# UZ-SLAMLab/DefSLAM

Measured on AMD Instinct MI355X. Metric: SfT GN iters/sec (500-node mesh, 1k matches), higher is better.
Workload: dtype f64

## Files before the change

### defslam_amd/csrc/sft_batch.h

```cpp
#pragma once

#define SFTB_NW 8
#ifndef SFTB_LIN_NW
#define SFTB_LIN_NW 8
#endif
#ifndef SFTB_LIN_WAVES
#define SFTB_LIN_WAVES 2
#endif
#ifndef SFTB_TRIAL_WAVES
#define SFTB_TRIAL_WAVES 2
#endif

__device__ __forceinline__ void sftb_ctl_lds(char* smem, Ctl*& ctl, double*& red, double*& out, double*& panel) {
  ctl = reinterpret_cast<Ctl*>(smem);
  red = reinterpret_cast<double*>(smem + 512);
  out = red + 16 * 27 + 5;
  panel = out + 32;
}

__global__ __launch_bounds__(64 * SFTB_NW, 2) void sftb_init_kernel(const SftDev* __restrict__ probs, SftRun* __restrict__ runs, int* __restrict__ counters, int* __restrict__ lin_list, int tail_below) {
  const SftDev& P = probs[blockIdx.x];
  if (blockIdx.x == 0 && threadIdx.x == 0 && (int)gridDim.x <= tail_below) counters[6] = 1;
  init_state<64 * SFTB_NW>(P);
  if (threadIdx.x == 0) {
    SftRun& R = runs[blockIdx.x];
    R.lambda = -1.0; R.ni = 2.0; R.chi_cur = 0.0; R.chi_ini = 0.0; R.rho = 0.0; R.lambda_start = 0.0;
    R.it = 0; R.qmax = 0; R.nbad = 0; R.accepted = 0; R.all_ok = 1; R.iters = 0; R.trials = 0; R.fact_ok = 1;
    R.state = P.max_iters > 0 ? SFTB_LIN : SFTB_FINISH;
    if (P.max_iters > 0) lin_list[atomicAdd(&counters[2], 1)] = blockIdx.x;
  }
}

template <int NW>
__device__ __forceinline__ void sftb_lin_problem(const SftDev& P, SftRun& R, Ctl* ctl, double* red, double* out, double* panel) {
  constexpr int NT = 64 * NW;
  const int tid = threadIdx.x;
  auto nothing = [] {};
  const double chi0 = linearise<NW, decltype(nothing), true>(P, ctl, red, out, panel, nothing);
  double lambda = R.lambda;
  if (R.it == 0) {
    double mx = 0.0;
    for (int r = tid; r < P.Dn; r += NT) mx = fmax(mx, fabs(h_diag(P, r)));
    if (tid < 6) mx = fmax(mx, fabs(P.Hcorner[tid * 8]));
    mx = block_max(mx, red);
    lambda = 1e-5 * mx;
  }
  if (tid == 0) {
    if (R.it == 0) { R.lambda = lambda; R.ni = 2.0; R.nbad = 0; }
    R.chi_cur = chi0; R.chi_ini = chi0; R.qmax = 0; R.rho = 0.0; R.accepted = 0; R.all_ok = 1; R.lambda_start = lambda;
    R.state = SFTB_TRIAL;
  }
}

__global__ __launch_bounds__(64 * SFTB_LIN_NW, SFTB_LIN_WAVES) void sftb_lin_kernel(const SftDev* __restrict__ probs, SftRun* __restrict__ runs, int* __restrict__ counters,
                                                                                  const int* __restrict__ lin_list, int B, int tail_below) {
  constexpr int NW = SFTB_LIN_NW, NT = 64 * NW;
  extern __shared__ __attribute__((aligned(16))) char smem[];
  __shared__ int next_b;
  Ctl* ctl; double *red, *out, *panel;
  sftb_ctl_lds(smem, ctl, red, out, panel);
  const int tid = threadIdx.x;
  if (counters[6] || B - counters[0] <= tail_below) {
    if (blockIdx.x == 0 && tid == 0) counters[6] = 1;
    return;
  }
  if (blockIdx.x == 0 && tid == 0) counters[7]++;
  auto fetch = [&]() { const int i = atomicAdd(&counters[3], 1); return i < counters[2] ? lin_list[i] : -1; };
  int nxt = -1;
  if (tid == 0) nxt = fetch();
  while (true) {
    if (tid == 0) next_b = nxt;
    __syncthreads();
    const int b = __builtin_amdgcn_readfirstlane(next_b);
    if (b < 0) break;
    if (tid == 0) { nxt = fetch(); atomicAdd(&counters[9], 1); }
    sftb_lin_problem<NW>(probs[b], runs[b], ctl, red, out, panel);
  }
}

__global__ __launch_bounds__(64, 1) void sftb_factor_kernel(const SftDev* __restrict__ probs, SftRun* __restrict__ runs, int* __restrict__ counters, int B) {
  extern __shared__ __attribute__((aligned(16))) char smem[];
  lds_double* lds = to_lds(reinterpret_cast<double*>(smem));
  const int lane = threadIdx.x;
  if (counters[6]) return;
  for (int i = lane; i < WV_LDS_DOUBLES; i += 64) lds[i] = 0.0;
  if (blockIdx.x == 0 && lane == 0) { counters[2] = 0; counters[3] = 0; }
  WvPrev Q;
  Q.Lg = nullptr; Q.Linv = nullptr; Q.x = nullptr; Q.nT = 0; Q.active = 0; Q.xb = 0.0;
  int n_done = 0;
  while (true) {
    int b = 0;
    if (lane == 0) b = atomicAdd(&counters[1], 1);
    b = __builtin_amdgcn_readfirstlane(b);
    if (b >= B) break;
    if (runs[b].state != SFTB_TRIAL) continue;
    const SftDev& P = probs[b];
    const double lambda = runs[b].lambda;
    double xcam;
    const int ok = wv_factor(P, lambda, lambda, lds, Q, xcam);
    if (lane == 0) runs[b].fact_ok = ok;
    Q = wv_prev_of(P, ok, xcam, lane);
    n_done++;
  }
  int lane_now;
  asm volatile("v_mbcnt_lo_u32_b32 %0, -1, 0\n\tv_mbcnt_hi_u32_b32 %0, -1, %0" : "=v"(lane_now));
  if (Q.active) wv_backsub_now(Q, lane_now);
  if (lane_now == 0 && n_done) atomicAdd(&counters[8], n_done);
}

template <int NW>
__device__ __forceinline__ int sftb_trial_problem(const SftDev& P, SftRun& R, Ctl* ctl, double* red, double* out, double* panel, int* counters, int* lin_list, int b) {
  constexpr int NT = 64 * NW;
  const int tid = threadIdx.x;
  const int Dn = P.Dn;
  const int Dnp = ((Dn + NB - 1) / NB) * NB;
  const int ok = R.fact_ok;
  const double lam = R.lambda;
  const bool in_lds = P.lds_class >= 1;
  if (!in_lds)
    for (int i = tid; i < 3 * P.n; i += NT) {
      const double v = P.xyz[i];
      P.xyz_bak[i] = v;
      const int a = P.act[i / 3];
      if (a >= 0) P.xyz[i] = v + P.x[3 * a + (i % 3)];
    }
  if (tid < 7) R.pose_bak[tid] = P.pose[tid];
  __syncthreads();
  if (tid == 0) pose_oplus(P.pose, P.x + Dnp);
  double sc = 0.0;
  for (int r = tid; r < Dn; r += NT) { const double xv = P.x[r]; sc += xv * (lam * xv + P.Hbord[(size_t)6 * Dnp + r]); }
  if (tid < 6) { const double xv = P.x[Dnp + tid]; sc += xv * (lam * xv + P.Hcorner[42 + tid]); }
  __syncthreads();
  block_sum<1>(&sc, red, out);
  const double scale = out[0];
  __syncthreads();
  const auto staged = asm_records<NW, 1>(P, panel);
  const double chi_new = in_lds ? eval_edges<false, 1>(P, ctl, red, out, staged, P.x)
                                : eval_edges<false, 0>(P, ctl, red, out, asm_records<NW, 0>(P, panel));
  if (tid == 0) {
    const double tempChi = ok ? chi_new : DBL_MAX;
    double rho = (R.chi_cur - tempChi);
    rho /= (scale + 1e-3);
    R.rho = rho;
    if (rho > 0 && isfinite(tempChi)) {
      double alpha = 1. - pow((2 * rho - 1), 3);
      alpha = fmin(alpha, 2. / 3.);
      const double sf = fmax(1. / 3., alpha);
      R.lambda = lam * sf; R.ni = 2.0; R.chi_cur = tempChi; R.accepted = 1;
      ctl->stop = 0;
    } else {
      R.lambda = lam * R.ni; R.ni *= 2.0;
      ctl->stop = 1;
    }
    R.qmax++;
    R.all_ok &= ok;
    ctl->qmax = R.qmax;
    ctl->rho = rho;
  }
  __syncthreads();
  if (ctl->stop) {
    if (!in_lds)
      for (int i = tid; i < 3 * P.n; i += NT) P.xyz[i] = P.xyz_bak[i];
    if (tid < 7) P.pose[tid] = R.pose_bak[tid];
  } else if (in_lds) {
    for (int i = tid; i < 3 * P.n; i += NT) P.xyz[i] = staged.xyz_l[i];
  }
  const bool again = (ctl->rho < 0) && (ctl->qmax < 10);
  if (again) return 0;
  __syncthreads();
  if (tid == 0) {
    const int qmax = R.qmax;
    R.trials += qmax;
    R.iters++;
    if (P.trace) {
      double* t = P.trace + R.it * 8;
      t[0] = R.chi_ini; t[1] = R.lambda_start; t[2] = qmax; t[3] = R.chi_cur; t[4] = R.lambda; t[5] = R.rho; t[6] = R.accepted; t[7] = R.all_ok;
    }
    if (!R.all_ok) P.res->status |= 1;
    bool term = (qmax == 10) || (R.rho == 0);
    if (!term) {
      if ((R.chi_ini - R.chi_cur) * 1e3 < R.chi_ini) R.nbad++; else R.nbad = 0;
      term = R.nbad >= 3;
    }
    R.it++;
    if (R.it >= P.max_iters) term = true;
    ctl->nbad = term ? 1 : 0;
    ctl->it = R.iters;
    ctl->accepted = R.trials;
    R.state = term ? SFTB_DONE : SFTB_LIN;
    if (!term && lin_list) lin_list[atomicAdd(&counters[2], 1)] = b;
  }
  __syncthreads();
  if (ctl->nbad) {
    const int iters = ctl->it, trials = ctl->accepted;
    __syncthreads();
    classify<NT>(P, ctl, panel, iters, trials);
    if (tid == 0) atomicAdd(&counters[0], 1);
    return 2;
  }
  return 1;
}

__global__ __launch_bounds__(64 * SFTB_NW, SFTB_TRIAL_WAVES) void sftb_trial_kernel(const SftDev* __restrict__ probs, SftRun* __restrict__ runs, int* __restrict__ counters, int* __restrict__ lin_list) {
  constexpr int NW = SFTB_NW, NT = 64 * NW;
  SftRun& R = runs[blockIdx.x];
  const int st = R.state;
  if (counters[6]) return;
  if (blockIdx.x == 0 && threadIdx.x == 0) counters[1] = 0;
  if (st != SFTB_TRIAL && st != SFTB_FINISH) return;
  extern __shared__ __attribute__((aligned(16))) char smem[];
  const SftDev& P = probs[blockIdx.x];
  Ctl* ctl; double *red, *out, *panel;
  sftb_ctl_lds(smem, ctl, red, out, panel);
  const int tid = threadIdx.x;
  if (st == SFTB_FINISH) {
    classify<NT>(P, ctl, panel, 0, 0);
    if (tid == 0) { R.state = SFTB_DONE; atomicAdd(&counters[0], 1); }
    return;
  }
  (void)sftb_trial_problem<NW>(P, R, ctl, red, out, panel, counters, lin_list, blockIdx.x);
}

__device__ __noinline__ void sftb_solve8(const SftDev& P, unsigned ctl_off, unsigned ws_off, double lambda) {
  typedef __attribute__((address_space(3))) char lds_char;
  Ctl* ctl = reinterpret_cast<Ctl*>((char*)(lds_char*)(size_t)__builtin_amdgcn_readfirstlane(ctl_off));
  double* ws = reinterpret_cast<double*>((char*)(lds_char*)(size_t)__builtin_amdgcn_readfirstlane(ws_off));
  factor_tiles_df8<1>(P, ctl, ws, lambda, true);
  backsub_tiles<8>(P, ctl, ws);
}

__global__ __launch_bounds__(64 * SFTB_NW, SFT_WAVES_PER_EU) void sftb_tail_kernel(const SftDev* __restrict__ probs, SftRun* __restrict__ runs, int* __restrict__ counters, int B, int tail_below) {
  constexpr int NW = SFTB_NW, NT = 64 * NW;
  extern __shared__ __attribute__((aligned(16))) char smem[];
  Ctl* ctl; double *red, *out, *panel;
  sftb_ctl_lds(smem, ctl, red, out, panel);
  const int tid = threadIdx.x;
  if (!counters[6]) {
    if (B - counters[0] > tail_below) return;
    if (blockIdx.x == 0 && tid == 0) counters[6] = 1;
  }
  while (true) {
    __syncthreads();
    if (tid == 0) ctl->it = atomicAdd(&counters[5], 1);
    __syncthreads();
    const int b = __builtin_amdgcn_readfirstlane(ctl->it);
    __syncthreads();
    if (b >= B) break;
    SftRun& R = runs[b];
    const SftDev& P = probs[b];
    int st = R.state;
    if (st == SFTB_FINISH) {
      classify<NT>(P, ctl, panel, 0, 0);
      if (tid == 0) { R.state = SFTB_DONE; atomicAdd(&counters[0], 1); }
      continue;
    }
    while (st == SFTB_LIN || st == SFTB_TRIAL) {
      if (st == SFTB_LIN) {
        sftb_lin_problem<NW>(P, R, ctl, red, out, panel);
        __syncthreads();
// ... 13 lines not shown
```

### defslam_amd/csrc/sft_wave.h

```cpp
#pragma once

#if defined(WV_STEP_TRACE) && defined(DSH_LAB)
#define WV_T_DECL long long wv_tr[9] = {0, 0, 0, 0, 0, 0, 0, 0, 0}, wv_tl = clock64()
#define WV_T(e) do { const long long t__ = clock64(); wv_tr[e] += t__ - wv_tl; wv_tl = t__; } while (0)
#define WV_T_ARG , long long (&wv_tr)[9], long long& wv_tl
#define WV_T_PASS , wv_tr, wv_tl
#define WV_T_DUMP(P) do { if ((threadIdx.x & 63) == 0) for (int e__ = 0; e__ < 9; e__++) (P).dbg[40 + e__] = (double)wv_tr[e__]; } while (0)
#else
#define WV_T_DECL do {} while (0)
#define WV_T(e) do {} while (0)
#define WV_T_ARG
#define WV_T_PASS
#define WV_T_DUMP(P) do {} while (0)
#endif

__host__ __device__ constexpr int wv_phys(int r, int d) {
  return d == 0 ? r : (d <= 3 ? 8 * d + r : (d == 4 ? 32 + (r & 3) : 8 * (8 - d) + ((r + 8 - d) & 7)));
}
constexpr int WV_AGPR_TILES = 32;
constexpr int WV_L_WIN = 0;
constexpr int WV_L_BORD = 1024;
constexpr int WV_L_WSCR = 2048;
constexpr int WV_L_CN = 2336;
constexpr int WV_L_XRING = 2400;
// ... 32 lines not shown
               "v_mfma_f64_16x16x4_f64 %0, %2, a[%c7:%c8], %0\n\t"
               "v_mfma_f64_16x16x4_f64 %0, %3, a[%c9:%c10], %0\n\t"
               "v_mfma_f64_16x16x4_f64 %0, %4, a[%c11:%c12], %0"
               : "=&v"(Y)
               : "v"(Wt[0]), "v"(Wt[1]), "v"(Wt[2]), "v"(Wt[3]), "i"(8 * T), "i"(8 * T + 1), "i"(8 * T + 2), "i"(8 * T + 3), "i"(8 * T + 4), "i"(8 * T + 5),
                 "i"(8 * T + 6), "i"(8 * T + 7)
               : "memory");
}
__device__ __forceinline__ void wv_trsm_vgpr(v4d& Y, const v4d& Wt, const v4d& D, int q0 = 0) {
  if (q0 <= 0) {
    asm volatile("s_nop 1\n\t"
                 "v_mfma_f64_16x16x4_f64 %0, %1, %5, 0\n\t"
                 "v_mfma_f64_16x16x4_f64 %0, %2, %6, %0\n\t"
                 "v_mfma_f64_16x16x4_f64 %0, %3, %7, %0\n\t"
                 "v_mfma_f64_16x16x4_f64 %0, %4, %8, %0"
                 : "=&v"(Y)
                 : "v"(Wt[0]), "v"(Wt[1]), "v"(Wt[2]), "v"(Wt[3]), "v"(D[0]), "v"(D[1]), "v"(D[2]), "v"(D[3])
                 : "memory");
  } else {
    asm volatile("s_nop 1\n\tv_mfma_f64_16x16x4_f64 %0, %1, %2, 0" : "=&v"(Y) : "v"(Wt[3]), "v"(D[3]) : "memory");
    if (q0 <= 2) asm volatile("v_mfma_f64_16x16x4_f64 %0, %1, %2, %0" : "+v"(Y) : "v"(Wt[2]), "v"(D[2]) : "memory");
    if (q0 <= 1) asm volatile("v_mfma_f64_16x16x4_f64 %0, %1, %2, %0" : "+v"(Y) : "v"(Wt[1]), "v"(D[1]) : "memory");
  }
}
struct WvTri { double a[10]; };
__device__ __forceinline__ void wv_tri_load(const lds_double* wscr, int lane, WvTri& A) {
  const lds_double* p = wscr + (lane & 3) * 17 + (lane >> 4);
#pragma unroll
  for (int q = 0; q < 4; q++)
#pragma unroll
    for (int k = 0; k <= q; k++) A.a[q * (q + 1) / 2 + k] = p[68 * q + 4 * k];
}
#define WV_TRI_BODY(D0, D1, D2, D3)                          \
  "v_mfma_f64_4x4x4_4b_f64 %3, %10, " D0 ", 0\n\t"   \
  "v_mfma_f64_4x4x4_4b_f64 %2, %7, " D0 ", 0\n\t"    \
  "v_mfma_f64_4x4x4_4b_f64 %3, %11, " D1 ", %3\n\t"  \
  "v_mfma_f64_4x4x4_4b_f64 %2, %8, " D1 ", %2\n\t"   \
  "v_mfma_f64_4x4x4_4b_f64 %3, %12, " D2 ", %3\n\t"  \
  "v_mfma_f64_4x4x4_4b_f64 %2, %9, " D2 ", %2\n\t"   \
  "v_mfma_f64_4x4x4_4b_f64 %3, %13, " D3 ", %3\n\t"  \
  "v_mfma_f64_4x4x4_4b_f64 %1, %5, " D0 ", 0\n\t"    \
  "v_mfma_f64_4x4x4_4b_f64 %0, %4, " D0 ", 0\n\t"    \
  "v_mfma_f64_4x4x4_4b_f64 %1, %6, " D1 ", %1"
template <int T>
__device__ __forceinline__ void wv_trsm4_agpr(v4d& Y, const WvTri& A) {
  asm volatile(WV_TRI_BODY("a[%c14:%c15]", "a[%c16:%c17]", "a[%c18:%c19]", "a[%c20:%c21]")
               : "=&v"(Y[0]), "=&v"(Y[1]), "=&v"(Y[2]), "=&v"(Y[3])
               : "v"(A.a[0]), "v"(A.a[1]), "v"(A.a[2]), "v"(A.a[3]), "v"(A.a[4]), "v"(A.a[5]), "v"(A.a[6]), "v"(A.a[7]), "v"(A.a[8]), "v"(A.a[9]),
                 "i"(8 * T), "i"(8 * T + 1), "i"(8 * T + 2), "i"(8 * T + 3), "i"(8 * T + 4), "i"(8 * T + 5), "i"(8 * T + 6), "i"(8 * T + 7)
               : "memory");
}
__device__ __forceinline__ void wv_trsm4_vgpr(v4d& Y, const WvTri& A, const v4d& D) {
  asm volatile("s_nop 1\n\t" WV_TRI_BODY("%14", "%15", "%16", "%17")
               : "=&v"(Y[0]), "=&v"(Y[1]), "=&v"(Y[2]), "=&v"(Y[3])
               : "v"(A.a[0]), "v"(A.a[1]), "v"(A.a[2]), "v"(A.a[3]), "v"(A.a[4]), "v"(A.a[5]), "v"(A.a[6]), "v"(A.a[7]), "v"(A.a[8]), "v"(A.a[9]),
                 "v"(D[0]), "v"(D[1]), "v"(D[2]), "v"(D[3])
               : "memory");
}
__device__ __forceinline__ void wv_trsm4_vgpr_q1(v4d& Y, const WvTri& A, const v4d& D) {
  asm volatile("s_nop 1\n\t"
               "v_mfma_f64_4x4x4_4b_f64 %2, %6, %9, 0\n\t"
               "v_mfma_f64_4x4x4_4b_f64 %1, %4, %9, 0\n\t"
               "v_mfma_f64_4x4x4_4b_f64 %2, %7, %10, %2\n\t"
               "v_mfma_f64_4x4x4_4b_f64 %1, %5, %10, %1\n\t"
               "v_mfma_f64_4x4x4_4b_f64 %2, %8, %11, %2\n\t"
               "v_mfma_f64_4x4x4_4b_f64 %0, %3, %9, 0"
               : "=&v"(Y[1]), "=&v"(Y[2]), "=&v"(Y[3])
               : "v"(A.a[2]), "v"(A.a[4]), "v"(A.a[5]), "v"(A.a[7]), "v"(A.a[8]), "v"(A.a[9]), "v"(D[1]), "v"(D[2]), "v"(D[3])
               : "memory");
  Y[0] = 0.0;
}
#undef WV_TRI_BODY
__device__ __forceinline__ void wv_mfma_fence() { asm volatile(WV_NOP_MFMA_RESULT ::: "memory"); }

template <int T>
__device__ __forceinline__ v4d wv_read_agpr() {
  int r[8];
  asm volatile("v_accvgpr_read_b32 %0, a[%c8]\n\tv_accvgpr_read_b32 %1, a[%c9]\n\tv_accvgpr_read_b32 %2, a[%c10]\n\tv_accvgpr_read_b32 %3, a[%c11]\n\t"
               "v_accvgpr_read_b32 %4, a[%c12]\n\tv_accvgpr_read_b32 %5, a[%c13]\n\tv_accvgpr_read_b32 %6, a[%c14]\n\tv_accvgpr_read_b32 %7, a[%c15]"
               : "=v"(r[0]), "=v"(r[1]), "=v"(r[2]), "=v"(r[3]), "=v"(r[4]), "=v"(r[5]), "=v"(r[6]), "=v"(r[7])
               : "i"(8 * T), "i"(8 * T + 1), "i"(8 * T + 2), "i"(8 * T + 3), "i"(8 * T + 4), "i"(8 * T + 5), "i"(8 * T + 6), "i"(8 * T + 7));
  v4d v;
#pragma unroll
  for (int q = 0; q < 4; q++) v[q] = __hiloint2double(r[2 * q + 1], r[2 * q]);
  return v;
}
template <int T>
__device__ __forceinline__ void wv_gather_agpr(const SFT_G double* base, unsigned o0, unsigned o1, unsigned o2, unsigned o3) {
  asm volatile("global_load_dwordx2 a[%c5:%c6], %0, %4\n\t"
               "global_load_dwordx2 a[%c7:%c8], %1, %4\n\t"
               "global_load_dwordx2 a[%c9:%c10], %2, %4\n\t"
               "global_load_dwordx2 a[%c11:%c12], %3, %4"
               :
               : "v"(o0), "v"(o1), "v"(o2), "v"(o3), "s"(base), "i"(8 * T), "i"(8 * T + 1), "i"(8 * T + 2), "i"(8 * T + 3), "i"(8 * T + 4), "i"(8 * T + 5),
                 "i"(8 * T + 6), "i"(8 * T + 7)
               : "memory");
}
template <int T, int Q>
__device__ __forceinline__ void wv_gather1_agpr(const SFT_G double* base, unsigned off) {
  asm volatile("global_load_dwordx2 a[%c2:%c3], %0, %1" : : "v"(off), "s"(base), "i"(8 * T + 2 * Q), "i"(8 * T + 2 * Q + 1) : "memory");
}
__device__ __forceinline__ void wv_wait_vm() { asm volatile("s_waitcnt vmcnt(0)" ::: "memory"); }

__device__ __forceinline__ v4d wv_lds_load(const lds_double* tile, int lane) {
  const lds_v2d* p = reinterpret_cast<const lds_v2d*>(tile);
  const v2d_w a = p[lane], b = p[64 + lane];
  return (v4d){a.x, a.y, b.x, b.y};
}
__device__ __forceinline__ void wv_lds_store(lds_double* tile, int lane, const v4d& v) {
  lds_v2d* p = reinterpret_cast<lds_v2d*>(tile);
  p[lane] = (v2d_w){v[0], v[1]};
  p[64 + lane] = (v2d_w){v[2], v[3]};
}
struct WvB2 { double n0, n1; };
struct WvBO { double v[4][2]; };
__device__ __forceinline__ WvB2 wv_bq_load(const lds_double* tile, int lane) {
  const v2d_w a = reinterpret_cast<const lds_v2d*>(tile)[lane];
  return WvB2{a.x, a.y};
}
__device__ __forceinline__ void wv_bq_store(lds_double* tile, int lane, const WvB2& v) {
  reinterpret_cast<lds_v2d*>(tile)[lane] = (v2d_w){v.n0, v.n1};
}
__device__ __forceinline__ int wv_bo_lane(int lane) { return (lane & 0x30) | (lane & 3); }
__device__ __forceinline__ void wv_bo_load(const lds_double* tile, int lane, WvBO& o) {
  const lds_v2d* p = reinterpret_cast<const lds_v2d*>(tile) + wv_bo_lane(lane);
#pragma unroll
  for (int q = 0; q < 4; q++) { const v2d_w a = p[4 * q]; o.v[q][0] = a.x; o.v[q][1] = a.y; }
}
__device__ __forceinline__ void wv_upd_b4(WvB2& C, const v4d& A, const WvBO& B, int q0 = 0) {
#define WV_MF(q) asm volatile("v_mfma_f64_4x4x4_4b_f64 %0, %2, %3, %0 neg:[1,0,0]\n\tv_mfma_f64_4x4x4_4b_f64 %1, %2, %4, %1 neg:[1,0,0]" \
                              : "+v"(C.n0), "+v"(C.n1) : "v"(A[q]), "v"(B.v[q][0]), "v"(B.v[q][1]) : "memory")
  asm volatile("s_nop 1" : "+v"(C.n0), "+v"(C.n1));
  if (q0 <= 0) WV_MF(0);
  if (q0 <= 1) WV_MF(1);
  if (q0 <= 2) WV_MF(2);
  WV_MF(3);
#undef WV_MF
}
__device__ __forceinline__ void wv_trsm_b4(WvB2& Y, const v4d& Wt, const WvBO& B) {
  asm volatile("s_nop 1\n\t"
               "v_mfma_f64_4x4x4_4b_f64 %0, %2, %6, 0\n\t"
               "v_mfma_f64_4x4x4_4b_f64 %1, %2, %7, 0\n\t"
               "v_mfma_f64_4x4x4_4b_f64 %0, %3, %8, %0\n\t"
               "v_mfma_f64_4x4x4_4b_f64 %1, %3, %9, %1\n\t"
               "v_mfma_f64_4x4x4_4b_f64 %0, %4, %10, %0\n\t"
               "v_mfma_f64_4x4x4_4b_f64 %1, %4, %11, %1\n\t"
               "v_mfma_f64_4x4x4_4b_f64 %0, %5, %12, %0\n\t"
               "v_mfma_f64_4x4x4_4b_f64 %1, %5, %13, %1"
               : "=&v"(Y.n0), "=&v"(Y.n1)
               : "v"(Wt[0]), "v"(Wt[1]), "v"(Wt[2]), "v"(Wt[3]), "v"(B.v[0][0]), "v"(B.v[0][1]), "v"(B.v[1][0]), "v"(B.v[1][1]), "v"(B.v[2][0]), "v"(B.v[2][1]),
                 "v"(B.v[3][0]), "v"(B.v[3][1])
               : "memory");
}
__device__ __forceinline__ int wv_bstd_index(int lane) { return 2 * wv_bo_lane(lane) + ((lane >> 2) & 1); }

template <int CTRL>
__device__ __forceinline__ double wv_dpp_mov(double v) {
  const int lo = __builtin_amdgcn_mov_dpp(__double2loint(v), CTRL, 0xF, 0xF, false);
  const int hi = __builtin_amdgcn_mov_dpp(__double2hiint(v), CTRL, 0xF, 0xF, false);
  return __hiloint2double(hi, lo);
}

__device__ __forceinline__ bool wv_chol_inv(v4d& a, v4d& w) {
  const int lane = threadIdx.x & 63;
  const int g = lane >> 4, c = lane & 15;
  w = (v4d){(g == c) ? 1.0 : 0.0, (g + 4 == c) ? 1.0 : 0.0, (g + 8 == c) ? 1.0 : 0.0, (g + 12 == c) ? 1.0 : 0.0};
  double plast = 1.0;
#pragma unroll
  for (int J = 0; J < 4; J++) {
    const double aJ = a[J];
    const double sel = chol4_inverse_operand(aJ, J, g, c & 3, plast);
    const double wJ = w[J];
    double zw, lp;
    if (J < 3) {
      asm volatile("s_nop 1\n\t"
                   "v_mfma_f64_4x4x4_4b_f64 %0, %2, %3, 0\n\t"
                   "v_mfma_f64_4x4x4_4b_f64 %1, %2, %4, 0\n\t"
                   "s_nop 7"
                   : "=&v"(zw), "=&v"(lp)
                   : "v"(sel), "v"(wJ), "v"(aJ));
      const double nlp = -lp;
      const double below = (c >= 4 * J + 4) ? nlp : 0.0;
      asm volatile("s_nop 1\n\t"
                   "v_mfma_f64_16x16x4_f64 %0, %2, %3, %0\n\t"
                   "v_mfma_f64_16x16x4_f64 %1, %4, %5, %1\n\t" WV_NOP_MFMA_RESULT
                   : "+v"(a), "+v"(w)
                   : "v"(nlp), "v"(lp), "v"(below), "v"(zw));
      w[J] = zw;
    } else {
      asm volatile("s_nop 1\n\tv_mfma_f64_4x4x4_4b_f64 %0, %1, %2, 0\n\ts_nop 7" : "=&v"(zw) : "v"(sel), "v"(wJ));
      w[J] = zw;
    }
  }
  return plast > 0.0;
}

struct WvProb {
  int Dn, Dnp, nT, q8;
  double lambda, lam_corner;
  unsigned bofs;
  const SFT_G double* Hc;
  const SFT_G uint32_t* hgl;
  const SFT_G double* Hbord;
  SFT_G double *Lg, *Linv;
};

typedef unsigned v4u_w __attribute__((ext_vector_type(4)));
__device__ __forceinline__ void wv_list(const WvProb& W, int I, int d, int lane, unsigned (&o)[4]) {
  const SFT_G v4u_w* row = reinterpret_cast<const SFT_G v4u_w*>(W.hgl + ((size_t)(I < W.nT ? I : W.nT) * (BT + 1) + d) * 256);
  const v4u_w v = row[lane];
  o[0] = v.x; o[1] = v.y; o[2] = v.z; o[3] = v.w;
}
__device__ __forceinline__ v4d wv_gather_vgpr(const WvProb& W, const unsigned (&o)[4]) {
  const auto b8 = reinterpret_cast<const SFT_G char*>(W.Hc);
  v4d v;
#pragma unroll
  for (int q = 0; q < 4; q++) v[q] = *reinterpret_cast<const SFT_G double*>(b8 + o[q]);
  return v;
}
__device__ __forceinline__ WvB2 wv_border_fresh(const WvProb& W, int J, int lane) {
  const SFT_G double* p = W.Hbord + TS * (J < W.nT ? J : W.nT);
  (void)lane;
  return WvB2{p[W.bofs], p[W.bofs + 4 * (unsigned)W.Dnp]};
}

struct WvRowList { unsigned o[8][4]; };
__device__ __forceinline__ void wv_row_list(const WvProb& W, int I, int lane, WvRowList& L) {
#pragma unroll
  for (int d = 0; d < 8; d++) wv_list(W, I, d, lane, L.o[d]);
}
template <int PH, int D>
__device__ __forceinline__ void wv_row_fetch_d(const WvProb& W, const WvRowList& L, int dmax, v4d& fresh4) {
  if constexpr (D < 8) {
    if (D <= dmax) {
      if constexpr (D == 4) fresh4 = wv_gather_vgpr(W, L.o[D]);
      else wv_gather_agpr<wv_phys(PH, D)>(W.Hc, L.o[D][0], L.o[D][1], L.o[D][2], L.o[D][3]);
    }
    wv_row_fetch_d<PH, D + 1>(W, L, dmax, fresh4);
  }
}

struct WvPrev {
  const SFT_G double* Lg;
  const SFT_G double* Linv;
  SFT_G double* x;
  int nT, active;
  double xb;
};
__device__ __forceinline__ void wv_bs_request(const WvPrev& Q, int J, lds_double* land, int lane) {
  const unsigned voff = 16u * (unsigned)lane;
  const SFT_G char* col = reinterpret_cast<const SFT_G char*>(Q.Lg + ((size_t)J * (BT + 1)) * 256);
  const SFT_G char* w = reinterpret_cast<const SFT_G char*>(Q.Linv + (size_t)J * 256);
  const unsigned l0 = (unsigned)__builtin_amdgcn_readfirstlane((int)(size_t)land);
  asm volatile("s_mov_b32 m0, %2\n\ts_nop 0\n\t"
               "global_load_lds_dwordx4 %0, %1\n\t"
               "global_load_lds_dwordx4 %0, %1 offset:2048\n\t"
               "global_load_lds_dwordx4 %0, %1 offset:3072"
               :: "v"(voff), "s"(col), "s"(l0) : "memory", "m0");
#pragma unroll
  for (int grp = 1; grp < 5; grp++) {
    const SFT_G char* cg = col + 4096 * grp;
    const unsigned lg = l0 + 4096u * grp;
    if (grp < 4)
      asm volatile("s_mov_b32 m0, %2\n\ts_nop 0\n\t"
                   "global_load_lds_dwordx4 %0, %1\n\t"
                   "global_load_lds_dwordx4 %0, %1 offset:1024\n\t"
                   "global_load_lds_dwordx4 %0, %1 offset:2048\n\t"
                   "global_load_lds_dwordx4 %0, %1 offset:3072"
                   :: "v"(voff), "s"(cg), "s"(lg) : "memory", "m0");
    else
      asm volatile("s_mov_b32 m0, %2\n\ts_nop 0\n\t"
                   "global_load_lds_dwordx4 %0, %1\n\t"
                   "global_load_lds_dwordx4 %0, %1 offset:1024"
                   :: "v"(voff), "s"(cg), "s"(lg) : "memory", "m0");
  }
  asm volatile("s_mov_b32 m0, %2\n\ts_nop 0\n\t"
               "global_load_lds_dwordx4 %0, %1\n\t"
               "global_load_lds_dwordx4 %0, %1 offset:1024"
               :: "v"(voff), "s"(w), "s"(l0 + 18u * 1024u) : "memory", "m0");
}
__device__ __forceinline__ void wv_bs_column(const WvPrev& Q, int J, const lds_double* land, lds_double* xring, int lane) {
  const int c = lane & 15;
  const lds_v2d* t2 = reinterpret_cast<const lds_v2d*>(land) + 2 * lane;
  double s[4];
  {
    const lds_double* tb = land + wv_bstd_index(lane);
    s[0] = tb[0] * Q.xb; s[1] = tb[8] * Q.xb; s[2] = tb[16] * Q.xb; s[3] = tb[24] * Q.xb;
  }
#pragma unroll
  for (int d = 1; d <= 8; d++) {
    const double xr = xring[((J + d) & 7) * 16 + c];
    const v2d_w a = t2[128 * d], b = t2[128 * d + 1];
    s[0] = fma(a.x, xr, s[0]); s[1] = fma(a.y, xr, s[1]); s[2] = fma(b.x, xr, s[2]); s[3] = fma(b.y, xr, s[3]);
  }
#pragma unroll
  for (int q = 0; q < 4; q++) {
    s[q] += wv_dpp_mov<0x128>(s[q]);
    s[q] += wv_dpp_mov<0x124>(s[q]);
    s[q] += wv_dpp_mov<0x122>(s[q]);
    s[q] += wv_dpp_mov<0x121>(s[q]);
  }
  const v2d_w wa = t2[128 * 9], wb = t2[128 * 9 + 1];
  double p = wa.x * -s[0];
  p = fma(wa.y, -s[1], p); p = fma(wb.x, -s[2], p); p = fma(wb.y, -s[3], p);
  p = sum_rows(p);
  if (lane < TS) { xring[(J & 7) * 16 + lane] = p; Q.x[TS * J + lane] = p; }
}
__device__ __forceinline__ void wv_bs_step(const WvPrev& Q, int J, lds_double* lds, int lane) {
  wv_bs_column(Q, J, lds + WV_L_LAND, lds + WV_L_XRING, lane);
  asm volatile("s_waitcnt lgkmcnt(0)" ::: "memory");
  if (J >= 1) wv_bs_request(Q, J - 1, lds + WV_L_LAND, lane);
}
__device__ __forceinline__ void wv_bs_begin(const WvPrev& Q, lds_double* lds, int lane) {
  lds_double* xring = lds + WV_L_XRING;
  xring[lane] = 0.0; xring[64 + lane] = 0.0;
  wv_bs_request(Q, Q.nT - 1, lds + WV_L_LAND, lane);
}
__device__ __forceinline__ void wv_backsub_now(const WvPrev& Q, int lane) {
  const int c = lane & 15;
  (void)c;
  double xr[8];
#pragma unroll
  for (int s = 0; s < 8; s++) xr[s] = 0.0;
  struct Col { v4d t[10]; };
  auto fetch = [&](int J) -> Col {
    Col C;
    if (J >= 0) {
      const SFT_G double* col = Q.Lg + ((size_t)J * (BT + 1)) * 256 + 4 * lane;
#pragma unroll
      for (int i = 1; i <= 8; i++) C.t[i] = (J + i < Q.nT) ? *reinterpret_cast<const SFT_G v4d*>(col + 256 * i) : (v4d){0.0, 0.0, 0.0, 0.0};
      {
        const SFT_G double* tb = col - 4 * lane + wv_bstd_index(lane);
        C.t[0] = (v4d){tb[0], tb[8], tb[16], tb[24]};
      }
      C.t[9] = *reinterpret_cast<const SFT_G v4d*>(Q.Linv + (size_t)J * 256 + 4 * lane);
    } else {
#pragma unroll
      for (int i = 0; i < 10; i++) C.t[i] = (v4d){0.0, 0.0, 0.0, 0.0};
    }
    return C;
  };
  auto solve_col = [&](const Col& C, int J, auto phc) {
    constexpr int ph = decltype(phc)::value;
    double s[4];
#pragma unroll
    for (int q = 0; q < 4; q++) s[q] = C.t[0][q] * Q.xb;
#pragma unroll
    for (int dd = 1; dd <= 8; dd++)
#pragma unroll
      for (int q = 0; q < 4; q++) s[q] = fma(C.t[dd][q], xr[(ph + dd) & 7], s[q]);
#pragma unroll
    for (int q = 0; q < 4; q++) {
      s[q] += wv_dpp_mov<0x128>(s[q]);
      s[q] += wv_dpp_mov<0x124>(s[q]);
      s[q] += wv_dpp_mov<0x122>(s[q]);
      s[q] += wv_dpp_mov<0x121>(s[q]);
    }
    double p = C.t[9][0] * -s[0];
#pragma unroll
    for (int q = 1; q < 4; q++) p = fma(C.t[9][q], -s[q], p);
    p = sum_rows(p);
    xr[ph] = p;
    if (lane < TS) Q.x[TS * J + lane] = p;
  };
  int J = Q.nT - 1;
  Col c0 = fetch(J), c1 = fetch(J - 1);
#pragma unroll 1
  for (; J >= 0; J -= 2) {
    const Col n0 = fetch(J - 2), n1 = fetch(J - 3);
    switch (J & 7) {
      case 7: solve_col(c0, J, std::integral_constant<int, 7>{}); solve_col(c1, J - 1, std::integral_constant<int, 6>{}); break;
      case 5: solve_col(c0, J, std::integral_constant<int, 5>{}); solve_col(c1, J - 1, std::integral_constant<int, 4>{}); break;
      case 3: solve_col(c0, J, std::integral_constant<int, 3>{}); solve_col(c1, J - 1, std::integral_constant<int, 2>{}); break;
      default: solve_col(c0, J, std::integral_constant<int, 1>{}); solve_col(c1, J - 1, std::integral_constant<int, 0>{}); break;
    }
    c0 = n0; c1 = n1;
  }
}

struct WvState {
  v4d Y[9];
  WvB2 Yq;
  WvBO Yo;
  double corner;
  v4d araw;
  WvB2 bnext;
  WvRowList rl;
  unsigned al[4];
  unsigned off_lane, off_bord;
  int ok;
};

template <int PH, int I, int IEND>
__device__ __forceinline__ void wv_trsm_cols(WvState& S, const WvTri& Wt, int k, int nT, const v4d& D4, int lane) {
  if constexpr (I <= IEND) {
    (void)k; (void)nT;
    if constexpr (I == 4) {
      wv_trsm4_vgpr(S.Y[4], Wt, D4);
    } else {
      wv_trsm4_agpr<wv_phys((PH + I) & 7, I)>(S.Y[I], Wt);
    }
    wv_trsm_cols<PH, I + 1, IEND>(S, Wt, k, nT, D4, lane);
  }
}

__host__ __device__ constexpr int wv_tile_index(int I, int J) {
  int n = 0;
  for (int i = 1; i <= 7; i++)
    for (int j = 1; j <= i; j++) {
      if (i == I && j == J) return n;
      if (i - j != 4) n++;
    }
  return n;
}
template <int PH, int SLOT>
__device__ __forceinline__ void wv_fetch_slot(const WvProb& W, const WvRowList& L) {
  if constexpr (SLOT < 28) {
    constexpr int t = SLOT / 4, q = SLOT % 4, d = t < 4 ? t : t + 1;
    wv_gather1_agpr<wv_phys(PH, d), q>(W.Hc, L.o[d][q]);
  }
}
template <int PH, bool TAIL, int I, int J>
__device__ __forceinline__ void wv_update_tiles(const WvProb& W, WvState& S, int k, int nT, int q8, SFT_G double* col) {
  if constexpr (I <= 8) {
    constexpr int d = I - J, r = (PH + I) & 7;
    if constexpr (d != 4) {
      if (!TAIL || k + I < nT) wv_upd_agpr<wv_phys(r, d)>(S.Y[J], S.Y[I], (I == 8) ? q8 : 0);
      if constexpr (I <= 7) {
        constexpr int n = wv_tile_index(I, J);
        if constexpr (n < 18) {
          const SFT_G double* slot = col + 256 * (n >> 1);
          if constexpr (n == 0) {
            const v2d_w yb = (v2d_w){S.Yq.n0, S.Yq.n1};
            asm volatile("global_store_dwordx4 %0, %1, %2" :: "v"(S.off_bord), "v"(yb), "s"(slot) : "memory");
          } else if constexpr (n >= 2) {
            const v4d& y = S.Y[n >> 1];
            const v2d_w half = (v2d_w){y[2 * (n & 1)], y[2 * (n & 1) + 1]};
            asm volatile("global_store_dwordx4 %0, %1, %2 offset:%c3" :: "v"(S.off_lane), "v"(half), "s"(slot), "n"(16 * (n & 1)) : "memory");
          }
        }
        wv_fetch_slot<PH, 2 * n>(W, S.rl);
        wv_fetch_slot<PH, 2 * n + 1>(W, S.rl);
      }
    }
    if constexpr (J < I) wv_update_tiles<PH, TAIL, I, J + 1>(W, S, k, nT, q8, col);
  }
}
template <int PH, bool TAIL, int I0, int I1>
__device__ __forceinline__ void wv_update_rows(const WvProb& W, WvState& S, int k, int nT, int q8, SFT_G double* col) {
  if constexpr (I0 <= I1) {
    wv_update_tiles<PH, TAIL, I0, 1>(W, S, k, nT, q8, col);
    wv_update_rows<PH, TAIL, I0 + 1, I1>(W, S, k, nT, q8, col);
  }
}
template <int PH, int T>
__device__ __forceinline__ lds_double* wv_task_tile(lds_double* lds) {
  if constexpr (T < 7) return lds + WV_L_BORD + 128 * ((PH + T + 1) & 7);
  else if constexpr (T < 10) return lds + WV_L_WIN + 256 * (wv_phys((PH + T - 2) & 7, 4) - WV_AGPR_TILES);
  else if constexpr (T == 10) return lds + WV_L_BORD + 128 * (PH & 7);
  else return lds + WV_L_WIN + 256 * (wv_phys(PH & 7, 4) - WV_AGPR_TILES);
}
template <int T> struct WvTaskTile { using type = typename std::conditional<(T < 7 || T == 10), WvB2, v4d>::type; };
template <int T> using wv_task_t = typename WvTaskTile<T>::type;
template <int PH, int T>
__device__ __forceinline__ wv_task_t<T> wv_task_load(lds_double* lds, int lane) {
  if constexpr (T < 7 || T == 10) return wv_bq_load(wv_task_tile<PH, T>(lds), lane);
  else return wv_lds_load(wv_task_tile<PH, T>(lds), lane);
}
template <int PH, int T>
__device__ __forceinline__ void wv_task_store(lds_double* lds, int lane, const wv_task_t<T>& C) {
  if constexpr (T < 7 || T == 10) wv_bq_store(wv_task_tile<PH, T>(lds), lane, C);
  else wv_lds_store(wv_task_tile<PH, T>(lds), lane, C);
}
template <int T>
__device__ __forceinline__ void wv_task_mfma(wv_task_t<T>& C, const WvState& S, int q8) {
  if constexpr (T < 7) wv_upd_b4(C, S.Y[T + 1], S.Yo);
  else if constexpr (T < 10) wv_upd_vgpr(C, S.Y[T - 6], S.Y[T - 2]);
  else if constexpr (T == 10) wv_upd_b4(C, S.Y[8], S.Yo, q8);
  else wv_upd_vgpr(C, S.Y[4], S.Y[8], q8);
}
template <int PH, int T, int TEND>
__device__ __forceinline__ void wv_lds_pipe_next(const WvState& S, int q8, lds_double* lds, int lane, wv_task_t<T>& C, const wv_task_t<T - 1>& Cprev) {
  if constexpr (T < TEND) {
    wv_task_t<T + 1> Cn = wv_task_load<PH, T + 1>(lds, lane);
    wv_task_mfma<T>(C, S, q8);
    wv_task_store<PH, T - 1>(lds, lane, Cprev);
    wv_lds_pipe_next<PH, T + 1, TEND>(S, q8, lds, lane, Cn, C);
  } else {
    wv_task_mfma<T>(C, S, q8);
    wv_task_store<PH, T - 1>(lds, lane, Cprev);
    wv_mfma_fence();
    wv_task_store<PH, T>(lds, lane, C);
  }
}
template <int PH, int T0, int TEND>
__device__ __forceinline__ void wv_lds_pipe(const WvState& S, int q8, lds_double* lds, int lane) {
  wv_task_t<T0> C = wv_task_load<PH, T0>(lds, lane);
  wv_task_t<T0 + 1> Cn = wv_task_load<PH, T0 + 1>(lds, lane);
  wv_task_mfma<T0>(C, S, q8);
  wv_lds_pipe_next<PH, T0 + 1, TEND>(S, q8, lds, lane, Cn, C);
}

template <int PH>
__device__ __forceinline__ v4d wv_step_diag(const WvProb& W, int k, int lane) {
  v4d d = wv_read_agpr<wv_phys(PH, 0)>();
  const int g = lane >> 4, c = lane & 15;
#pragma unroll
  for (int q = 0; q < 4; q++)
    if (g + 4 * q == c && TS * k + c < W.Dn) d[q] += W.lambda;
  return d;
}

template <int PH, bool TAIL>
__device__ __forceinline__ void wv_step_rest(const WvProb& W, WvState& S, const v4d& w, int k, lds_double* lds, int lane, const WvPrev& Q WV_T_ARG) {
  lds_double* ldsw = lds + WV_L_WIN;
  lds_double* ldsb = lds + WV_L_BORD;
  lds_double* wscr = lds + WV_L_WSCR;
  const int nT = W.nT;
  WvBO Bk;
  wv_bo_load(ldsb + 128 * PH, lane, Bk);
  const v4d D4 = wv_lds_load(ldsw + 256 * (wv_phys((PH + 4) & 7, 4) - WV_AGPR_TILES), lane);
  v4d Wt;
  {
    const int g = lane >> 4, c = lane & 15;
#pragma unroll
    for (int q = 0; q < 4; q++) wscr[(g + 4 * q) * 17 + c] = w[q];
#pragma unroll
    for (int q = 0; q < 4; q++) Wt[q] = wscr[c * 17 + g + 4 * q];
  }
  WvTri Wq;
  wv_tri_load(wscr, lane, Wq);
  WV_T(2);
// ... 99 lines not shown
#ifdef DSH_LAB
  const long long wv_t0 = clock64();
#endif
  if (Q.active) wv_bs_begin(Q, lds, lane);
  WvState S;
#pragma unroll
  for (int i = 0; i < 9; i++) S.Y[i] = (v4d){0.0, 0.0, 0.0, 0.0};
  const int cr = 4 * (c >> 3) + g, cc = 4 * ((c >> 2) & 1) + (c & 3);
  S.corner = 0.0;
  if (cr < SFT_BORDER && cc < SFT_BORDER && cc <= cr) S.corner = P.Hcorner[cr * 7 + cc] + ((cr == cc && cr < 6) ? lam_corner : 0.0);
  S.ok = 1;
  {
    WvTriList T;
    v4d f4[8];
    WvB2 bd[8];
    wv_prologue_lists<0, 0>(W, lane, T);
    wv_prologue_gathers<0, 0>(W, T, f4);
#pragma unroll
    for (int r = 0; r < 8; r++) bd[r] = wv_border_fresh(W, r, lane);
    wv_list(W, 8, 8, lane, S.al);
    wv_prologue_store<0>(lds, lane, f4[0], bd[0]); wv_prologue_store<1>(lds, lane, f4[1], bd[1]); wv_prologue_store<2>(lds, lane, f4[2], bd[2]);
    wv_prologue_store<3>(lds, lane, f4[3], bd[3]); wv_prologue_store<4>(lds, lane, f4[4], bd[4]); wv_prologue_store<5>(lds, lane, f4[5], bd[5]);
    wv_prologue_store<6>(lds, lane, f4[6], bd[6]); wv_prologue_store<7>(lds, lane, f4[7], bd[7]);
  }
  wv_wait_vm();
  asm volatile("" : "+v"(S.al[0]), "+v"(S.al[1]), "+v"(S.al[2]), "+v"(S.al[3]));
#ifdef DSH_LAB
  const long long wv_t1 = clock64();
  const long long wv_w1 = wall_clock64();
#endif

  WV_T_DECL;
#pragma unroll 1
  for (int k = 0; k < W.nT; k++) {
    const int ph = k & 7;
    asm volatile("v_lshlrev_b32 %0, 5, %1" : "=v"(S.off_lane) : "v"(lane));
    asm volatile("v_lshlrev_b32 %0, 4, %1" : "=v"(S.off_bord) : "v"(lane));
    S.araw = wv_gather_vgpr(W, S.al);
    wv_list(W, k + 9, 8, lane, S.al);
    wv_row_list(W, k + 8, lane, S.rl);
    S.bnext = wv_border_fresh(W, k + 8, lane);
    v4d d;
    switch (ph) {
      case 0: d = wv_step_diag<0>(W, k, lane); break;
      case 1: d = wv_step_diag<1>(W, k, lane); break;
      case 2: d = wv_step_diag<2>(W, k, lane); break;
      case 3: d = wv_step_diag<3>(W, k, lane); break;
      case 4: d = wv_step_diag<4>(W, k, lane); break;
      case 5: d = wv_step_diag<5>(W, k, lane); break;
      case 6: d = wv_step_diag<6>(W, k, lane); break;
      default: d = wv_step_diag<7>(W, k, lane); break;
    }
    WV_T(0);
    if (Q.active) {
      const int J = Q.nT - 1 - k;
      if (J >= 0) wv_bs_step(Q, J, lds, lane);
    }
    WV_T(7);
    v4d w;
    if (!wv_chol_inv(d, w)) {
#ifdef DSH_LAB
      if (S.ok && lane == 0) P.dbg[3] = 1000.0 + k;
#endif
      S.ok = 0;
    }
    WV_T(1);
    {
      const SFT_G double* slot = W.Linv + (size_t)k * 256;
      const v2d_w w01 = (v2d_w){w[0], w[1]}, w23 = (v2d_w){w[2], w[3]};
      asm volatile("global_store_dwordx4 %0, %1, %3\n\tglobal_store_dwordx4 %0, %2, %3 offset:16" :: "v"(S.off_lane), "v"(w01), "v"(w23), "s"(slot) : "memory");
    }
    switch (ph + ((k + 8 >= W.nT) ? 8 : 0)) {
      case 0: wv_step_rest<0, false>(W, S, w, k, lds, lane, Q WV_T_PASS); break;
      case 1: wv_step_rest<1, false>(W, S, w, k, lds, lane, Q WV_T_PASS); break;
      case 2: wv_step_rest<2, false>(W, S, w, k, lds, lane, Q WV_T_PASS); break;
      case 3: wv_step_rest<3, false>(W, S, w, k, lds, lane, Q WV_T_PASS); break;
      case 4: wv_step_rest<4, false>(W, S, w, k, lds, lane, Q WV_T_PASS); break;
      case 5: wv_step_rest<5, false>(W, S, w, k, lds, lane, Q WV_T_PASS); break;
      case 6: wv_step_rest<6, false>(W, S, w, k, lds, lane, Q WV_T_PASS); break;
      case 7: wv_step_rest<7, false>(W, S, w, k, lds, lane, Q WV_T_PASS); break;
      case 8: wv_step_rest<0, true>(W, S, w, k, lds, lane, Q WV_T_PASS); break;
      case 9: wv_step_rest<1, true>(W, S, w, k, lds, lane, Q WV_T_PASS); break;
      case 10: wv_step_rest<2, true>(W, S, w, k, lds, lane, Q WV_T_PASS); break;
      case 11: wv_step_rest<3, true>(W, S, w, k, lds, lane, Q WV_T_PASS); break;
      case 12: wv_step_rest<4, true>(W, S, w, k, lds, lane, Q WV_T_PASS); break;
      case 13: wv_step_rest<5, true>(W, S, w, k, lds, lane, Q WV_T_PASS); break;
      case 14: wv_step_rest<6, true>(W, S, w, k, lds, lane, Q WV_T_PASS); break;
      default: wv_step_rest<7, true>(W, S, w, k, lds, lane, Q WV_T_PASS); break;
    }
  }
  WV_T_DUMP(P);
  if (Q.active) {
    for (int J = Q.nT - 1 - W.nT; J >= 0; J--) { wv_wait_vm(); wv_bs_step(Q, J, lds, lane); }
  }
#ifdef DSH_LAB
  const long long wv_t2 = clock64();
  const long long wv_w2 = wall_clock64();
#endif
  wv_mfma_fence();
  {
    int l2;
    asm volatile("v_mbcnt_lo_u32_b32 %0, -1, 0\n\tv_mbcnt_hi_u32_b32 %0, -1, %0" : "=v"(l2));
    const int g2 = l2 >> 4, c2 = l2 & 15;
    const int cr2 = 4 * (c2 >> 3) + g2, cc2 = 4 * ((c2 >> 2) & 1) + (c2 & 3);
    if (cr2 < SFT_BORDER && cc2 < SFT_BORDER) Cn[cr2 * 7 + cc2] = S.corner;
  }
  double xcam = 0.0;
  {
    int okc = 1;
    if (lane == 0) {
      double xc[6] = {0, 0, 0, 0, 0, 0};
      bool bad = false;
      for (int kk = 0; kk < 6; kk++) {
        double dd = Cn[kk * 7 + kk];
        for (int j = 0; j < kk; j++) dd -= Cn[kk * 7 + j] * Cn[kk * 7 + j];
        if (!(dd > 0.0)) bad = true;
        const double piv = sqrt(dd);
        Cn[kk * 7 + kk] = piv;
        for (int r = kk + 1; r < 7; r++) {
          double v = Cn[r * 7 + kk];
          for (int j = 0; j < kk; j++) v -= Cn[r * 7 + j] * Cn[kk * 7 + j];
          Cn[r * 7 + kk] = v / piv;
        }
      }
      if (bad) okc = 0;
      for (int kk = 5; kk >= 0; kk--) {
        double v = Cn[6 * 7 + kk];
        for (int r = kk + 1; r < 6; r++) v -= Cn[r * 7 + kk] * xc[r];
        xc[kk] = v / Cn[kk * 7 + kk];
      }
      for (int kk = 0; kk < 6; kk++) Cn[49 + kk] = xc[kk];
    }
    okc = __builtin_amdgcn_readfirstlane(okc);
    if (!okc) S.ok = 0;
    if (c < 6) xcam = Cn[49 + c];
  }
  xcam_out = xcam;
#ifdef DSH_LAB
  if (lane == 0) { P.dbg[5] = (double)(wv_t1 - wv_t0); P.dbg[6] = (double)(wv_t2 - wv_t1); P.dbg[4] = (double)(wv_w2 - wv_w1); }
#endif
  return __builtin_amdgcn_readfirstlane(S.ok);
}

__device__ __forceinline__ WvPrev wv_prev_of(const SftDev& P, int ok, double xcam, int lane_) {
  (void)lane_;
  int lane;
  asm volatile("v_mbcnt_lo_u32_b32 %0, -1, 0\n\tv_mbcnt_hi_u32_b32 %0, -1, %0" : "=v"(lane));
  const int c = lane & 15;
  WvPrev Q;
  const int Dn = uni(P.Dn), Dnp = ((Dn + NB - 1) / NB) * NB;
  Q.Lg = uni(P.Lb); Q.Linv = uni(P.Linv); Q.x = uni(P.x);
  Q.nT = Dnp / TS;
  Q.active = ok;
  Q.xb = (c < 6) ? xcam : ((c == 6) ? -1.0 : 0.0);
  if (ok && lane < 6) P.x[Dnp + lane] = xcam;
  return Q;
}

__device__ __forceinline__ int wv_factor_solve(const SftDev& P, double lambda, double lam_corner, lds_double* lds) {
  WvPrev none;
  none.Lg = nullptr; none.Linv = nullptr; none.x = nullptr; none.nT = 0; none.active = 0; none.xb = 0.0;
  double xcam;
  const int ok = wv_factor(P, lambda, lam_corner, lds, none, xcam);
  int lane;
  asm volatile("v_mbcnt_lo_u32_b32 %0, -1, 0\n\tv_mbcnt_hi_u32_b32 %0, -1, %0" : "=v"(lane));
  const WvPrev Q = wv_prev_of(P, ok, xcam, lane);
#ifdef DSH_LAB
  const long long t2 = clock64();
#endif
  if (ok) wv_backsub_now(Q, lane);
#ifdef DSH_LAB
  if (lane == 0) P.dbg[7] = (double)(clock64() - t2);
#endif
  return ok;
}
```

Before: 420,500.

## Restructure wave back-substitution to cut cross-lane reductions via transposed tile layout

Rewrites the per-column back-substitution so each lane gathers a transposed slice of the L tile and the solution ring is kept in LDS instead of registers. The four 16-lane DPP reduction trees become a single two-step reduction, and the Linv product uses v_fmac_f64_dpp row broadcasts. The border term is split into two per-lane values so it needs no extra shuffles. This trades reduction depth and the phase-specialised switch for extra LDS traffic and scattered, uncoalesced global loads in the prefetch path.

Result: no change. 421,600, median of 6 (+0.3%).

```diff
diff --git a/defslam_amd/csrc/sft_batch.h b/defslam_amd/csrc/sft_batch.h
--- a/defslam_amd/csrc/sft_batch.h
+++ b/defslam_amd/csrc/sft_batch.h
@@ -86,7 +86,7 @@
   for (int i = lane; i < WV_LDS_DOUBLES; i += 64) lds[i] = 0.0;
   if (blockIdx.x == 0 && lane == 0) { counters[2] = 0; counters[3] = 0; }
   WvPrev Q;
-  Q.Lg = nullptr; Q.Linv = nullptr; Q.x = nullptr; Q.nT = 0; Q.active = 0; Q.xb = 0.0;
+  Q.Lg = nullptr; Q.Linv = nullptr; Q.x = nullptr; Q.nT = 0; Q.active = 0; Q.xb0 = 0.0; Q.xb1 = 0.0;
   int n_done = 0;
   while (true) {
     int b = 0;
@@ -104,7 +104,7 @@
   }
   int lane_now;
   asm volatile("v_mbcnt_lo_u32_b32 %0, -1, 0\n\tv_mbcnt_hi_u32_b32 %0, -1, %0" : "=v"(lane_now));
-  if (Q.active) wv_backsub_now(Q, lane_now);
+  if (Q.active) wv_backsub_now(Q, lds, lane_now);
   if (lane_now == 0 && n_done) atomicAdd(&counters[8], n_done);
 }
 
diff --git a/defslam_amd/csrc/sft_wave.h b/defslam_amd/csrc/sft_wave.h
--- a/defslam_amd/csrc/sft_wave.h
+++ b/defslam_amd/csrc/sft_wave.h
@@ -208,7 +208,6 @@
                  "v"(B.v[3][0]), "v"(B.v[3][1])
                : "memory");
 }
-__device__ __forceinline__ int wv_bstd_index(int lane) { return 2 * wv_bo_lane(lane) + ((lane >> 2) & 1); }
 
 template <int CTRL>
 __device__ __forceinline__ double wv_dpp_mov(double v) {
@@ -301,7 +300,7 @@
   const SFT_G double* Linv;
   SFT_G double* x;
   int nT, active;
-  double xb;
+  double xb0, xb1;
 };
 __device__ __forceinline__ void wv_bs_request(const WvPrev& Q, int J, lds_double* land, int lane) {
   const unsigned voff = 16u * (unsigned)lane;
@@ -335,32 +334,60 @@
                "global_load_lds_dwordx4 %0, %1 offset:1024"
                :: "v"(voff), "s"(w), "s"(l0 + 18u * 1024u) : "memory", "m0");
 }
+constexpr int WV_BS_XB = 128;
+__device__ __forceinline__ int wv_bs_tidx(int lane) { return 4 * (lane & 0x33) + ((lane >> 2) & 3); }
+__device__ __forceinline__ void wv_bs_ring_load(const lds_double* xring, int slot, int lane, double (&x)[4]) {
+  const lds_v2d* p = reinterpret_cast<const lds_v2d*>(xring + 16 * slot) + 2 * (lane & 3);
+  const v2d_w a = p[0], b = p[1];
+  x[0] = a.x; x[1] = a.y; x[2] = b.x; x[3] = b.y;
+}
+__device__ __forceinline__ double wv_bs_rowsum(const double (&t)[8][4], const double (&x)[8][4], const v2d_w& yb, const v2d_w& xb) {
+  double s0 = yb.x * xb.x, s1 = yb.y * xb.y, s2 = t[0][2] * x[0][2], s3 = t[0][3] * x[0][3];
+  s0 = fma(t[0][0], x[0][0], s0);
+  s1 = fma(t[0][1], x[0][1], s1);
+#pragma unroll
+  for (int d = 1; d < 8; d++) {
+    s0 = fma(t[d][0], x[d][0], s0);
+    s1 = fma(t[d][1], x[d][1], s1);
+    s2 = fma(t[d][2], x[d][2], s2);
+    s3 = fma(t[d][3], x[d][3], s3);
+  }
+  double s = (s0 + s1) + (s2 + s3);
+  s += wv_dpp_mov<0xB1>(s);
+  s += wv_dpp_mov<0x4E>(s);
+  return s;
+}
+__device__ __forceinline__ double wv_bs_wprod(double s, const v4d& w) {
+  double p = 0.0;
+  asm volatile("s_nop 1\n\t"
+               "v_fmac_f64_dpp %0, -%1, %2 row_newbcast:0 row_mask:0xf bank_mask:0xf\n\t"
+               "v_fmac_f64_dpp %0, -%1, %3 row_newbcast:4 row_mask:0xf bank_mask:0xf\n\t"
+               "v_fmac_f64_dpp %0, -%1, %4 row_newbcast:8 row_mask:0xf bank_mask:0xf\n\t"
+               "v_fmac_f64_dpp %0, -%1, %5 row_newbcast:12 row_mask:0xf bank_mask:0xf"
+               : "+v"(p)
+               : "v"(s), "v"(w[0]), "v"(w[1]), "v"(w[2]), "v"(w[3]));
+  return sum_rows(p);
+}
+__device__ __forceinline__ void wv_bs_result(const WvPrev& Q, int J, lds_double* xring, int lane, double p) {
+  if (lane < TS) {
+    xring[(J & 7) * 16 + 4 * (lane & 3) + (lane >> 2)] = p;
+    Q.x[TS * J + lane] = p;
+  }
+}
 __device__ __forceinline__ void wv_bs_column(const WvPrev& Q, int J, const lds_double* land, lds_double* xring, int lane) {
-  const int c = lane & 15;
-  const lds_v2d* t2 = reinterpret_cast<const lds_v2d*>(land) + 2 * lane;
-  double s[4];
-  {
-    const lds_double* tb = land + wv_bstd_index(lane);
-    s[0] = tb[0] * Q.xb; s[1] = tb[8] * Q.xb; s[2] = tb[16] * Q.xb; s[3] = tb[24] * Q.xb;
-  }
+  const lds_double* tl = land + wv_bs_tidx(lane);
+  double t[8][4], x[8][4];
 #pragma unroll
   for (int d = 1; d <= 8; d++) {
-    const double xr = xring[((J + d) & 7) * 16 + c];
-    const v2d_w a = t2[128 * d], b = t2[128 * d + 1];
-    s[0] = fma(a.x, xr, s[0]); s[1] = fma(a.y, xr, s[1]); s[2] = fma(b.x, xr, s[2]); s[3] = fma(b.y, xr, s[3]);
-  }
-#pragma unroll
-  for (int q = 0; q < 4; q++) {
-    s[q] += wv_dpp_mov<0x128>(s[q]);
-    s[q] += wv_dpp_mov<0x124>(s[q]);
-    s[q] += wv_dpp_mov<0x122>(s[q]);
-    s[q] += wv_dpp_mov<0x121>(s[q]);
-  }
-  const v2d_w wa = t2[128 * 9], wb = t2[128 * 9 + 1];
-  double p = wa.x * -s[0];
-  p = fma(wa.y, -s[1], p); p = fma(wb.x, -s[2], p); p = fma(wb.y, -s[3], p);
-  p = sum_rows(p);
-  if (lane < TS) { xring[(J & 7) * 16 + lane] = p; Q.x[TS * J + lane] = p; }
+    wv_bs_ring_load(xring, (J + d) & 7, lane, x[d - 1]);
+#pragma unroll
+    for (int j = 0; j < 4; j++) t[d - 1][j] = tl[256 * d + 16 * j];
+  }
+  const v2d_w yb = reinterpret_cast<const lds_v2d*>(land)[lane];
+  const v2d_w xb = reinterpret_cast<const lds_v2d*>(land + WV_BS_XB)[lane & 3];
+  const lds_v2d* w2 = reinterpret_cast<const lds_v2d*>(land + 256 * 9) + 2 * lane;
+  const v2d_w wa = w2[0], wb = w2[1];
+  wv_bs_result(Q, J, xring, lane, wv_bs_wprod(wv_bs_rowsum(t, x, yb, xb), (v4d){wa.x, wa.y, wb.x, wb.y}));
 }
 __device__ __forceinline__ void wv_bs_step(const WvPrev& Q, int J, lds_double* lds, int lane) {
   wv_bs_column(Q, J, lds + WV_L_LAND, lds + WV_L_XRING, lane);
@@ -370,70 +397,51 @@
 __device__ __forceinline__ void wv_bs_begin(const WvPrev& Q, lds_double* lds, int lane) {
   lds_double* xring = lds + WV_L_XRING;
   xring[lane] = 0.0; xring[64 + lane] = 0.0;
+  if (lane < 4) reinterpret_cast<lds_v2d*>(lds + WV_L_LAND + WV_BS_XB)[lane] = (v2d_w){Q.xb0, Q.xb1};
   wv_bs_request(Q, Q.nT - 1, lds + WV_L_LAND, lane);
 }
-__device__ __forceinline__ void wv_backsub_now(const WvPrev& Q, int lane) {
-  const int c = lane & 15;
-  (void)c;
-  double xr[8];
-#pragma unroll
-  for (int s = 0; s < 8; s++) xr[s] = 0.0;
-  struct Col { v4d t[10]; };
+__device__ __forceinline__ void wv_backsub_now(const WvPrev& Q, lds_double* lds, int lane) {
+  lds_double* xring = lds + WV_L_XRING;
+  xring[lane] = 0.0; xring[64 + lane] = 0.0;
+  const int tix = wv_bs_tidx(lane);
+  const v2d_w xb = (v2d_w){Q.xb0, Q.xb1};
+  struct Col { double t[8][4]; v2d_w yb; v4d w; };
   auto fetch = [&](int J) -> Col {
     Col C;
     if (J >= 0) {
-      const SFT_G double* col = Q.Lg + ((size_t)J * (BT + 1)) * 256 + 4 * lane;
-#pragma unroll
-      for (int i = 1; i <= 8; i++) C.t[i] = (J + i < Q.nT) ? *reinterpret_cast<const SFT_G v4d*>(col + 256 * i) : (v4d){0.0, 0.0, 0.0, 0.0};
-      {
-        const SFT_G double* tb = col - 4 * lane + wv_bstd_index(lane);
-        C.t[0] = (v4d){tb[0], tb[8], tb[16], tb[24]};
-      }
-      C.t[9] = *reinterpret_cast<const SFT_G v4d*>(Q.Linv + (size_t)J * 256 + 4 * lane);
+      const SFT_G double* col = Q.Lg + ((size_t)J * (BT + 1)) * 256;
+#pragma unroll
+      for (int i = 1; i <= 8; i++)
+#pragma unroll
+        for (int j = 0; j < 4; j++) C.t[i - 1][j] = (J + i < Q.nT) ? col[256 * i + tix + 16 * j] : 0.0;
+      C.yb = reinterpret_cast<const SFT_G v2d_w*>(col)[lane];
+      C.w = *reinterpret_cast<const SFT_G v4d*>(Q.Linv + (size_t)J * 256 + 4 * lane);
     } else {
 #pragma unroll
-      for (int i = 0; i < 10; i++) C.t[i] = (v4d){0.0, 0.0, 0.0, 0.0};
+      for (int i = 0; i < 8; i++)
+#pragma unroll
+        for (int j = 0; j < 4; j++) C.t[i][j] = 0.0;
+      C.yb = (v2d_w){0.0, 0.0};
+      C.w = (v4d){0.0, 0.0, 0.0, 0.0};
     }
     return C;
   };
-  auto solve_col = [&](const Col& C, int J, auto phc) {
-    constexpr int ph = decltype(phc)::value;
-    double s[4];
-#pragma unroll
-    for (int q = 0; q < 4; q++) s[q] = C.t[0][q] * Q.xb;
-#pragma unroll
-    for (int dd = 1; dd <= 8; dd++)
-#pragma unroll
-      for (int q = 0; q < 4; q++) s[q] = fma(C.t[dd][q], xr[(ph + dd) & 7], s[q]);
-#pragma unroll
-    for (int q = 0; q < 4; q++) {
-      s[q] += wv_dpp_mov<0x128>(s[q]);
-      s[q] += wv_dpp_mov<0x124>(s[q]);
-      s[q] += wv_dpp_mov<0x122>(s[q]);
-      s[q] += wv_dpp_mov<0x121>(s[q]);
-    }
-    double p = C.t[9][0] * -s[0];
-#pragma unroll
-    for (int q = 1; q < 4; q++) p = fma(C.t[9][q], -s[q], p);
-    p = sum_rows(p);
-    xr[ph] = p;
-    if (lane < TS) Q.x[TS * J + lane] = p;
+  auto solve_col = [&](const Col& C, int J) {
+    double x[8][4];
+#pragma unroll
+    for (int d = 1; d <= 8; d++) wv_bs_ring_load(xring, (J + d) & 7, lane, x[d - 1]);
+    wv_bs_result(Q, J, xring, lane, wv_bs_wprod(wv_bs_rowsum(C.t, x, C.yb, xb), C.w));
   };
   int J = Q.nT - 1;
   Col c0 = fetch(J), c1 = fetch(J - 1);
 #pragma unroll 1
   for (; J >= 0; J -= 2) {
     const Col n0 = fetch(J - 2), n1 = fetch(J - 3);
-    switch (J & 7) {
-      case 7: solve_col(c0, J, std::integral_constant<int, 7>{}); solve_col(c1, J - 1, std::integral_constant<int, 6>{}); break;
-      case 5: solve_col(c0, J, std::integral_constant<int, 5>{}); solve_col(c1, J - 1, std::integral_constant<int, 4>{}); break;
-      case 3: solve_col(c0, J, std::integral_constant<int, 3>{}); solve_col(c1, J - 1, std::integral_constant<int, 2>{}); break;
-      default: solve_col(c0, J, std::integral_constant<int, 1>{}); solve_col(c1, J - 1, std::integral_constant<int, 0>{}); break;
-    }
+    solve_col(c0, J);
+    solve_col(c1, J - 1);
     c0 = n0; c1 = n1;
   }
 }
-
 struct WvState {
   v4d Y[9];
   WvB2 Yq;
@@ -839,14 +847,16 @@
   Q.Lg = uni(P.Lb); Q.Linv = uni(P.Linv); Q.x = uni(P.x);
   Q.nT = Dnp / TS;
   Q.active = ok;
-  Q.xb = (c < 6) ? xcam : ((c == 6) ? -1.0 : 0.0);
+  const double xb = (c < 6) ? xcam : ((c == 6) ? -1.0 : 0.0);
+  Q.xb0 = __shfl(xb, lane & 3);
+  Q.xb1 = __shfl(xb, 4 + (lane & 3));
   if (ok && lane < 6) P.x[Dnp + lane] = xcam;
   return Q;
 }
 
 __device__ __forceinline__ int wv_factor_solve(const SftDev& P, double lambda, double lam_corner, lds_double* lds) {
   WvPrev none;
-  none.Lg = nullptr; none.Linv = nullptr; none.x = nullptr; none.nT = 0; none.active = 0; none.xb = 0.0;
+  none.Lg = nullptr; none.Linv = nullptr; none.x = nullptr; none.nT = 0; none.active = 0; none.xb0 = 0.0; none.xb1 = 0.0;
   double xcam;
   const int ok = wv_factor(P, lambda, lam_corner, lds, none, xcam);
   int lane;
@@ -855,7 +865,7 @@
 #ifdef DSH_LAB
   const long long t2 = clock64();
 #endif
-  if (ok) wv_backsub_now(Q, lane);
+  if (ok) wv_backsub_now(Q, lds, lane);
 #ifdef DSH_LAB
   if (lane == 0) P.dbg[7] = (double)(clock64() - t2);
 #endif
```
